# imgag/ngs-bits

Hardware: AMD Instinct MI355X
Metric: Mreads/sec + achieved HBM GB/s, MappingQC 30x WGS BAM at 1/2/4/8 MI355X (higher is better)
Workload: dtype u8/int32/int64

## Files before the change

### ngs-bits_amd/csrc/handle.h

```cpp
#pragma once
#include "common.h"
#include <memory>
#include <condition_variable>
#include <mutex>
#include <algorithm>
#include <cstring>
#include <chrono>
#include <atomic>
#include <functional>
#include <thread>
#include <deque>
#include <fstream>
#include <fcntl.h>
#include <sys/mman.h>
#include <sys/stat.h>
#include <unistd.h>

using namespace ngsqc;

namespace ngsqc { namespace lib {
extern thread_local std::string g_open_error;

struct FormatError : std::runtime_error { using std::runtime_error::runtime_error; };
struct ArgError : std::runtime_error { using std::runtime_error::runtime_error; };
// ... 99 lines not shown

inline uint16_t rd16(const uint8_t* p) { return (uint16_t)(p[0] | (p[1] << 8)); }
inline uint32_t rd32(const uint8_t* p) { return (uint32_t)p[0] | ((uint32_t)p[1] << 8) | ((uint32_t)p[2] << 16) | ((uint32_t)p[3] << 24); }

constexpr int K1_CHUNK_WAVES_PER_CU = 5;
constexpr int P1_WAVES_PER_CU = 10;
constexpr int N_DEPTH_SETS = 2;

struct DepthSet
{
	std::vector<ngsqc_region> regions; std::vector<int64_t> doff; std::vector<int32_t> rlen; int64_t n_slots = 0; int64_t roi_bases = 0;
	DevBuf<int32_t> d_reg_start, d_reg_end, d_reg_len, d_tid_first, d_tid_last; DevBuf<int64_t> d_doff; DevBuf<int32_t> d_depth; DevBuf<uint8_t> d_tmp;
	bool depth_ready = false;
};

struct TileCtx { const uint8_t* infl; int64_t total; const int64_t* recoff; int64_t n_rec; int64_t ord_base; int tile; bool last; };
}}

using namespace ngsqc::lib;

struct ngsqc_handle
{
	const OpenSwitches osw;
	CallSwitches sw;
	std::string err, path;
	bool from_cram = false;
	bool selection = false;
	int device = 0; int n_cu = 256;
	hipStream_t stream = nullptr;
	hipStream_t s_p1[2] = {nullptr, nullptr};
	hipStream_t s_p2 = nullptr;
	hipStream_t s_crc = nullptr;
	size_t csize = 0;
	std::vector<BlockDesc> blocks; int64_t total = 0;
	std::vector<uint32_t> crc;
	std::vector<uint64_t> member_off;
	DevBuf<uint8_t> d_comp;
	std::vector<std::string> ref_names; std::vector<int64_t> ref_lens; int64_t first_rec = 0; std::string header_text;
	bool planned = false;
	int64_t chunk = 0, nch = 0;
	std::vector<std::pair<int64_t, int64_t>> tiles;
	std::vector<int64_t> tile_first_chunk;
	int64_t pfx = 0, max_tile_bytes = 0, slot_pages = 0;
	DevBuf<BlockDesc> d_kdesc;
	DevBuf<uint32_t> d_tok_first, d_tok_cnt, d_order, d_tok, d_crc, d_pool_ctr; DevBuf<unsigned long long> d_work; DevBuf<BlockStatus> d_status;
	int p1_wgs = 0;
	DevBuf<uint32_t> d_sync_pool; DevBuf<BlockDesc> d_sync_desc; DevBuf<uint32_t> d_sync_u32; DevBuf<BlockStatus> d_sync_st; DevBuf<unsigned long long> d_sync_work;
	static constexpr int MAX_TILE_BUFS = 4;
	int k1_slots = osw.token_slots;
	DevBuf<uint8_t> buf[MAX_TILE_BUFS]; int nbuf = 2;
	int64_t max_tile_members = 0;
	std::vector<hipEvent_t> ev_chunk;
	std::vector<hipEvent_t> ev_tile;
	PinBuf<BlockStatus> p_status; PinBuf<int32_t> p_start; PinBuf<int64_t> p_next; PinBuf<unsigned long long> p_small;
	bool decoded = false; int cur_tile = -1;
	int64_t n_rec = 0; DevBuf<int64_t> d_recoff;
	DevBuf<int64_t> d_long;
	int64_t tile_prefix = 0, tile_total = 0, tile_u_lo = 0, tile_ord_base = 0;
	int64_t carry_len = 0, carry_src = 0, next_ord_base = 0, expected_abs = 0;
	int64_t k1_enq = 0;
	DevBuf<int32_t> d_start; DevBuf<uint32_t> d_cnt; DevBuf<int64_t> d_next, d_base; DevBuf<uint32_t> d_bad; DevBuf<uint8_t> d_scan_tmp; DevBuf<uint16_t> d_rel;
	DepthSet ds[N_DEPTH_SETS]; int cur_ds = 0;
	ngsqc_timings tm{};
	int shard = 0, n_shards = 1;
	int64_t shard_own_members = -1;
	int64_t shard_limit = -1;
	int64_t shard_u_base = 0;
	int64_t shard_first_abs = -1, shard_exit_abs = -1; int shard_last_tile = -1;
	bool verify_crc = osw.verify_crc;
	struct Upload
	{
		std::vector<std::thread> th; std::mutex mu; std::condition_variable cv;
		std::vector<hipEvent_t> ev; std::vector<char> recorded; size_t piece = 0, n_pieces = 0, bytes = 0; std::atomic<size_t> next{0}; std::atomic<bool> cancel{false};
		std::string err; void* map = nullptr; size_t map_n = 0; int fd = -1; double t0 = 0, t_done = 0; size_t done = 0;
		size_t waited[4] = {0, 0, 0, 0};
		struct SPiece { size_t src, dst, bytes; int64_t chunk; };
		std::vector<SPiece> sp; std::vector<size_t> chunk_first;
		std::atomic<int64_t> p2_enq{0}; bool pass_running = false, pass_fresh = false; const uint8_t* src_base = nullptr;
	};
	Upload* up = nullptr;
	bool stream_img = false; int comp_slots = 0; size_t comp_slot_bytes = 0;
	std::vector<uint64_t> chunk_lo;
	DevBuf<uint8_t> d_sync_comp;
	std::thread plan_thread; std::string plan_err;
	EvLog ev_store; EvLog* evlog = &ev_store;
	PinBuf<unsigned long long> p_rb; static constexpr int RB_CAND = 64, RB_BQ = 65, RB_TOTAL = 72;
	bool lazy_recoff = false; int recoff_tile = -1;
	struct RecoffArgs { const uint8_t* base = nullptr; int64_t total = 0; const BlockDesc* desc = nullptr; int64_t ne = 0, prefix = 0, n_rec = 0, nm = 0; int ksh = 0; int tile = -1; } rw;
	struct FusedScan
	{
		virtual void fused_launch(ngsqc_handle* h, const uint8_t* infl, int64_t total, int sgn, const BlockDesc* d_desc, int64_t ne, int64_t prefix, int ksh, int64_t nm, int64_t scan_limit) = 0;
		virtual void fused_readback(ngsqc_handle* h) = 0;
		virtual unsigned long long fused_bq_cap() = 0;
		virtual ~FusedScan() = default;
	};
	FusedScan* fuse = nullptr; bool fuse_ok = true; int fused_tile = -1;
	bool long_reads = false;
	int lr_failures = 0;
	bool k2_plain = false;
	std::vector<int64_t> rq_len_hist, rq_cyc;
	struct Partial;
	Partial* partial = nullptr;
};

namespace ngsqc { namespace lib {
inline void dbg_stamp(bool on, const char* what)
{
	static const double t0 = wall_ms();
	if (on) fprintf(stderr, "[ngsqc] t+%.1f ms %s\n", wall_ms() - t0, what);
}

template <typename F> int guarded(ngsqc_handle* h, F f)
{
	if (!h) return NGSQC_E_ARG;
	h->sw = CallSwitches();
	try { HIPCHK(hipSetDevice(h->device)); f(); return NGSQC_OK; }
	catch (FormatError& e) { h->err = e.what(); return NGSQC_E_FORMAT; }
	catch (ArgError& e) { h->err = e.what(); return NGSQC_E_ARG; }
	catch (IoError& e) { h->err = e.what(); return NGSQC_E_IO; }
	catch (std::domain_error& e) { h->err = e.what(); return NGSQC_E_UNSUPPORTED; }
	catch (std::exception& e) { h->err = e.what(); return NGSQC_E_DEVICE; }
}

void walk_bgzf(const uint8_t* file, size_t n, size_t& off, size_t off_end, int64_t max_members, uint64_t& upos, std::vector<BlockDesc>& blocks, std::vector<uint32_t>& crc, std::vector<uint64_t>* file_off = nullptr);
void scan_bgzf(const uint8_t* file, size_t n, std::vector<BlockDesc>& blocks, std::vector<uint32_t>& crc, int64_t& total, std::vector<uint64_t>* file_off, int threads, bool* in_pieces = nullptr);
std::string inflate_error(const ngsqc_handle* h, int64_t member, uint32_t code);
void inflate_sync(ngsqc_handle* h, const std::vector<int64_t>& idx, const std::vector<BlockDesc>& desc, uint8_t* d_out, int level = 0);
void upload_wait(ngsqc_handle* h, size_t end_byte, hipStream_t st, int slot);
void upload_join(ngsqc_handle* h);
void upload_finish(ngsqc_handle* h);
void stream_pass_begin(ngsqc_handle* h);
void stream_pass_end(ngsqc_handle* h);
void stream_wait_chunk(ngsqc_handle* h, int64_t c, hipStream_t st);
void stream_p2_enqueued(ngsqc_handle* h, int64_t c);
void plan_layout(ngsqc_handle* h);
struct RangeRequest { bool by_name = false; uint64_t voff[2] = {0, 0}; const ngsqc_named_region* regions = nullptr; int64_t n_regions = 0; int64_t head_members = 0; };
int open_impl(ngsqc_handle** out, const char* path, const void* bytes, size_t n, int device, int shard = 0, int n_shards = 1, const RangeRequest* range = nullptr);

const int64_t* ensure_recoff(ngsqc_handle* h);
void sync_all(ngsqc_handle* h);
void stream_tiles(ngsqc_handle* h, const std::function<bool(const TileCtx&)>& f);
void for_each_tile(ngsqc_handle* h, const std::function<bool(int)>& f);

constexpr int64_t BGZF_PIECE = 0xff00;
size_t bgzf_max_bytes(int64_t n);
struct BgzfDeflater
{
	DevBuf<uint16_t> prev; DevBuf<uint32_t> tok, sizes; DevBuf<uint64_t> off; DevBuf<uint8_t> slots, scan_tmp;
	int grid = 0; int64_t cap_members = 0;
	void reserve(int64_t max_members, int device);
	size_t run(const uint8_t* d_in, int64_t n, uint8_t* d_out, hipStream_t s, int device, int level = -1);
// ... 5 lines not shown
```

### ngs-bits_amd/csrc/image.hip

```cpp
#include "handle.h"

namespace ngsqc { namespace lib {
void walk_bgzf(const uint8_t* file, size_t n, size_t& off, size_t off_end, int64_t max_members, uint64_t& upos, std::vector<BlockDesc>& blocks, std::vector<uint32_t>& crc, std::vector<uint64_t>* file_off)
{
	int64_t k = 0;
	while (off < n && off < off_end && k < max_members)
	{
		if (off + 18 > n) throw FormatError("truncated BGZF header");
		const uint8_t* p = file + off;
		if (p[0] != 31 || p[1] != 139 || p[2] != 8 || !(p[3] & 4)) throw FormatError("not a BGZF block (gzip member without BC extra field)");
		uint32_t xlen = rd16(p + 10), bsize = 0; bool found = false;
		size_t x = 12, xend = 12 + (size_t)xlen;
		if (off + xend > n) throw FormatError("truncated BGZF extra field");
		while (x + 4 <= xend) { uint16_t slen = rd16(p + x + 2); if (p[x] == 'B' && p[x + 1] == 'C' && slen == 2) { bsize = rd16(p + x + 4) + 1u; found = true; } x += 4 + slen; }
		if (!found || bsize < xend + 8 || off + bsize > n) throw FormatError("invalid BGZF block size");
		uint32_t isize = rd32(p + bsize - 4);
		if (isize > 65536) throw FormatError("BGZF block inflates to more than 64 KiB");
		if (isize) { blocks.push_back(BlockDesc{(uint64_t)(off + xend), upos, (uint32_t)(bsize - xend - 8), isize}); crc.push_back(rd32(p + bsize - 8)); if (file_off) file_off->push_back((uint64_t)off); }
		upos += isize; off += bsize; ++k;
	}
}
uint32_t bgzf_member_at(const uint8_t* file, size_t n, size_t off)
{
	if (off + 18 > n) return 0;
// ... 469 lines not shown
	}
	if (h->nch <= cpt) cpt = h->nch;
	h->tiles.clear(); h->tile_first_chunk.clear();
	for (int64_t c = 0; c < h->nch; c += cpt)
	{
		const int64_t m0 = c * h->chunk, m1 = std::min(nb, (c + cpt) * h->chunk);
		h->tiles.emplace_back(m0, m1 - m0); h->tile_first_chunk.push_back(c);
	}
	h->tile_first_chunk.push_back(h->nch);
	const int nt = (int)h->tiles.size();
	h->pfx = nt > 1 ? ((carry_max + 255) & ~255ll) : 0;
	std::vector<BlockDesc> kd((size_t)nb); h->max_tile_bytes = 0;
	for (int t = 0; t < nt; ++t)
	{
		const int64_t f = h->tiles[(size_t)t].first, m = h->tiles[(size_t)t].second; const uint64_t u_lo = h->blocks[(size_t)f].upos;
		for (int64_t i = f; i < f + m; ++i) { kd[(size_t)i] = h->blocks[(size_t)i]; kd[(size_t)i].upos -= u_lo; }
		h->max_tile_bytes = std::max<int64_t>(h->max_tile_bytes, (int64_t)(h->blocks[(size_t)(f + m - 1)].upos + h->blocks[(size_t)(f + m - 1)].usize - u_lo));
	}
	if (h->stream_img)
	{
		h->comp_slots = (int)std::min<int64_t>(h->osw.comp_slots ? h->osw.comp_slots : 8, h->nch);
		h->chunk_lo.assign((size_t)h->nch, 0); std::vector<uint64_t> chunk_hi((size_t)h->nch, 0); size_t slot = 0;
		for (int64_t c = 0; c < h->nch; ++c)
		{
			const int64_t c0 = c * h->chunk, cn = std::min(h->chunk, nb - c0);
			h->chunk_lo[(size_t)c] = h->blocks[(size_t)c0].cpos & ~15ull;
			chunk_hi[(size_t)c] = std::min<uint64_t>(h->blocks[(size_t)(c0 + cn - 1)].cpos + h->blocks[(size_t)(c0 + cn - 1)].clen + 64, h->up->map_n);
			slot = std::max<size_t>(slot, (size_t)(chunk_hi[(size_t)c] - h->chunk_lo[(size_t)c]));
		}
		h->comp_slot_bytes = (slot + 1024 + 4095) & ~(size_t)4095;
		h->d_comp.alloc((size_t)h->comp_slots * h->comp_slot_bytes + 1024);
		HIPCHK(hipMemsetAsync(h->d_comp.p, 0, (size_t)h->comp_slots * h->comp_slot_bytes + 1024, h->stream));
		const size_t piece = (size_t)h->osw.h2d_piece_mb << 20;
		ngsqc_handle::Upload* u = h->up; u->sp.clear(); u->chunk_first.assign((size_t)h->nch + 1, 0);
		for (int64_t c = 0; c < h->nch; ++c)
		{
			const int64_t c0 = c * h->chunk, cn = std::min(h->chunk, nb - c0);
			const size_t base = (size_t)(c % h->comp_slots) * h->comp_slot_bytes;
			for (int64_t i = c0; i < c0 + cn; ++i) kd[(size_t)i].cpos = base + (h->blocks[(size_t)i].cpos - h->chunk_lo[(size_t)c]);
			u->chunk_first[(size_t)c] = u->sp.size();
			for (uint64_t o = h->chunk_lo[(size_t)c]; o < chunk_hi[(size_t)c]; o += piece)
				u->sp.push_back(ngsqc_handle::Upload::SPiece{(size_t)o, base + (size_t)(o - h->chunk_lo[(size_t)c]), (size_t)std::min<uint64_t>(piece, chunk_hi[(size_t)c] - o), c});
		}
		u->chunk_first[(size_t)h->nch] = u->sp.size();
	}
	h->d_kdesc.upload(kd, h->stream); h->d_order.upload(ord, h->stream); h->d_crc.upload(h->crc, h->stream);
	h->d_tok_cnt.ensure((size_t)nb + 8); h->d_tok_first.ensure((size_t)nb + 8); h->d_status.ensure((size_t)nb); h->d_work.ensure((size_t)h->nch); h->d_pool_ctr.ensure((size_t)h->nch);
	dbg_stamp(h->osw.debug, "layout: member tables on the device");
	h->d_tok.ensure((size_t)(n_slots * h->slot_pages) * K1_PAGE_WORDS + 16);
	dbg_stamp(h->osw.debug, "layout: token pool allocated");
	for (int i = 0; i < std::min(nt, h->nbuf); ++i) h->buf[i].ensure((size_t)(h->pfx + h->max_tile_bytes) + 64);
	dbg_stamp(h->osw.debug, "layout: tile buffers allocated");
	h->max_tile_members = 0; for (auto& tl : h->tiles) h->max_tile_members = std::max(h->max_tile_members, tl.second);
	h->p_status.ensure((size_t)nb);
	while ((int64_t)h->ev_chunk.size() < 4 * h->nch) { hipEvent_t e; HIPCHK(hipEventCreate(&e)); h->ev_chunk.push_back(e); }
	while ((int)h->ev_tile.size() < 2 * nt) { hipEvent_t e; HIPCHK(hipEventCreateWithFlags(&e, hipEventDisableTiming)); h->ev_tile.push_back(e); }
	h->p_small.ensure(64); h->p_rb.ensure((size_t)ngsqc_handle::RB_TOTAL);
	HIPCHK(hipStreamSynchronize(h->stream));
	h->tm.n_tiles = nt;
	if (h->stream_img && early_pass) { stream_pass_begin(h); h->up->pass_fresh = true; }
	if (h->osw.debug) fprintf(stderr, "[ngsqc] layout: %d tiles, %lld chunks, %d image slots, token pool %.1f GB, tile buffers %.1f GB, %.1f ms\n", nt, (long long)h->nch, h->comp_slots, (double)n_slots * (double)h->slot_pages * K1_PAGE_WORDS * 4e-9, (double)std::min(nt, h->nbuf) * (double)(h->pfx + h->max_tile_bytes) * 1e-9, wall_ms() - pl0);
}

void plan_layout(ngsqc_handle* h)
{
	if (h->plan_thread.joinable())
	{
		h->plan_thread.join();
		if (!h->plan_err.empty()) { const std::string e = h->plan_err; h->plan_err.clear(); throw std::runtime_error(e); }
	}
	plan_layout_now(h);
}


void open_range_common(ngsqc_handle* h, const uint8_t* bytes, size_t n, int device, const RangeRequest& rq)
{
	if (n >= 4 && memcmp(bytes, "CRAM", 4) == 0) throw std::domain_error("a CRAM file has no BGZF members: ngsqc_open / ngsqc_open_memory decode it (cram.hip)");
	init_device(h, device);
	Timer t(h->stream); t.start();
	size_t off = 0; uint64_t upos = 0; std::vector<uint64_t> hdr_off;
	for (int64_t k = 8;; k *= 4)
	{
		walk_bgzf(bytes, n, off, n, k - (int64_t)hdr_off.size() > 0 ? k - (int64_t)hdr_off.size() : k, upos, h->blocks, h->crc, &hdr_off);
		const size_t end = h->blocks.empty() ? 0 : (size_t)(h->blocks.back().cpos + h->blocks.back().clen);
		upload_compressed(h, bytes, 0, end);
		h->total = (int64_t)upos;
		if (read_header(h, (int64_t)h->blocks.size())) break;
		if (off >= n) throw FormatError("Could not read header from BAM/CRAM file " + h->path);
	}
	uint64_t beg = rq.voff[0], end = rq.voff[1]; bool found = true;
	uint64_t own_end = 0;
	if (rq.by_name)
	{
		std::vector<ngsqc_region> regs;
		for (int64_t i = 0; i < rq.n_regions; ++i)
		{
			const std::string want = rq.regions[i].chr ? rq.regions[i].chr : "";
			for (size_t r = 0; r < h->ref_names.size(); ++r) if (h->ref_names[r] == want || chr_norm(h->ref_names[r]) == chr_norm(want)) { regs.push_back(ngsqc_region{(int32_t)r, rq.regions[i].start, rq.regions[i].end}); break; }
		}
		if (!bai_range(h->path, regs.data(), (int64_t)regs.size(), (int32_t)h->ref_names.size(), beg, end, found))
			throw IoError("Could not load index of BAM/CRAM file " + h->path);
	}
	if (rq.head_members > 0)
	{
		size_t k = 0; while (k + 1 < h->blocks.size() && (int64_t)(h->blocks[k].upos + h->blocks[k].usize) <= h->first_rec) ++k;
		found = !h->blocks.empty() && h->first_rec < h->total;
		if (!found && off < n) { walk_bgzf(bytes, n, off, n, 1, upos, h->blocks, h->crc, &hdr_off); h->total = (int64_t)upos; k = h->blocks.size() - 1; found = h->first_rec < h->total; }
// ... 127 lines not shown
```

### ngs-bits_amd/csrc/jobs.hip

```cpp
#include "handle.h"

namespace ngsqc { namespace lib {

void setup_regions(ngsqc_handle* h, DepthSet& D, const ngsqc_region* regions, int64_t n, bool with_depth = true)
{
	const int n_ref = (int)h->ref_names.size();
	D.regions.assign(regions, regions + (n > 0 ? n : 0));
	D.doff.assign((size_t)n + 1, 0); D.rlen.assign((size_t)n, 0);
	std::vector<int32_t> rs((size_t)n), re((size_t)n), tf((size_t)std::max(n_ref, 1), 0), tl((size_t)std::max(n_ref, 1), 0);
	std::vector<uint8_t> seen((size_t)std::max(n_ref, 1), 0);
	int64_t slots = 0, bases = 0;
	for (int64_t i = 0; i < n; ++i)
	{
		const ngsqc_region& r = regions[i];
		if (r.tid < 0 || r.tid >= n_ref) throw ArgError("region with invalid reference id");
		if (r.start < 1 || r.end < r.start) throw ArgError("invalid region range");
		if (i > 0 && regions[i - 1].tid == r.tid) { if (regions[i - 1].end >= r.start) throw ArgError("Merged and sorted BED file required for coverage details statistics!"); }
		else { if (seen[r.tid]) throw ArgError("Merged and sorted BED file required for coverage details statistics!"); seen[r.tid] = 1; tf[r.tid] = (int32_t)i; }
		tl[r.tid] = (int32_t)i + 1;
		rs[i] = r.start; re[i] = r.end; D.rlen[i] = r.end - r.start + 1; D.doff[i] = slots;
		slots += (int64_t)D.rlen[i] + 1; bases += D.rlen[i];
	}
	D.doff[n] = slots; D.n_slots = slots; D.roi_bases = bases;
	D.d_reg_start.upload(rs, h->stream); D.d_reg_end.upload(re, h->stream); D.d_reg_len.upload(D.rlen, h->stream);
// ... 627 lines not shown
	{
		map.scan.end(h);
		if (!part)
		{
			Timer fin(h->stream); fin.start();
			finalize_depth(h, h->ds[0]);
			h->tm.finalize_ms = fin.stop();
			mapping_counters(h, map, (int)(map.scan.best_key >> 40), map.scan.first_paired != ~0ull, map.scan.sum_runmax, map.scan.fix_len, r->counters, r->gc_reads);
		}
		else
		{
			const unsigned long long key = map.scan.best_key;
			shard_out->n_records = h->tm.n_records;
			shard_out->first_abs = h->shard_own_members >= 0 ? h->shard_first_abs : (h->tm.n_records ? h->first_rec : -1);
			shard_out->exit_abs = h->shard_own_members >= 0 ? h->shard_exit_abs : (h->tm.n_records ? h->total : -1);
			shard_out->max_len = (int64_t)(key >> 40);
			shard_out->first_max_ord = key ? (int64_t)(0xFFFFFFFFFFull - (key & 0xFFFFFFFFFFull)) : -1;
			shard_out->first_paired_ord = map.scan.first_paired != ~0ull ? (int64_t)map.scan.first_paired : -1;
		}
		h->tm.scan_ms = map.scan.stage_ms; h->tm.scan_kernel_ms = map.scan.kernel_ms; h->tm.scan_launches = map.scan.launches;
	}
	if (do_depth)
	{
		dscan.end(h);
		if (!part) { Timer fin(h->stream); fin.start(); finalize_depth(h, h->ds[1]); h->tm.finalize_ms += fin.stop(); }
		h->tm.depth_scan_ms = dscan.stage_ms;
		if (!do_map) { h->tm.scan_algorithmic_bytes = (int64_t)dscan.dev[A_ALG_BYTES]; h->tm.scan_kernel_ms = dscan.kernel_ms; h->tm.scan_launches = dscan.launches; h->tm.scan_ms = dscan.stage_ms; }
	}
	if (do_sites) { pile.end(h, r->site_counts); h->tm.pileup_ms = pile.stage_ms; }
	if (do_indel) { indel.end(h, ij->counts); h->tm.pileup_ms += indel.stage_ms; }
	if (do_reads) { reads.end(h, r->read_stats); h->tm.reads_ms = reads.stage_ms; }
	h->cur_ds = do_map || !do_depth ? 0 : 1;
	h->tm.total_ms = total.stop();
	h->tm.job_wall_ms = wall_ms() - w0;
	if (h->sw.debug) fprintf(stderr, "[ngsqc] job: setup %.2f ms, tile stream %.2f ms (K1 %.2f), results %.2f ms\n", w1 - w0, w2 - w1, h->tm.inflate_ms, wall_ms() - w2);
}

DepthSet& cur_depth(ngsqc_handle* h) { return h->ds[h->cur_ds]; }

}}

extern "C" {

void ngsqc_close(ngsqc_handle* h)
{
	if (!h) return;
	struct Hold { Hold() { reaper().hold(); } ~Hold() { reaper().unhold(); } } hold_frees;
	if (h->plan_thread.joinable()) h->plan_thread.join();
	if (h->up) { upload_join(h); delete h->up; h->up = nullptr; }
	if (h->stream) { (void)hipSetDevice(h->device); sync_all(h); }
	for (hipStream_t s : {h->stream, h->s_p1[0], h->s_p1[1], h->s_p2, h->s_crc}) if (s) (void)hipStreamDestroy(s);
	for (hipEvent_t e : h->ev_chunk) (void)hipEventDestroy(e);
	for (hipEvent_t e : h->ev_tile) (void)hipEventDestroy(e);
	delete h->partial;
	delete h;
}

int ngsqc_run_job(ngsqc_handle* h, const ngsqc_job_desc* job, ngsqc_job_result* result) { return guarded(h, [&] { run_job(h, job, result); }); }

int ngsqc_depth_select(ngsqc_handle* h, int32_t which)
{
	return guarded(h, [&] { if (which < 0 || which >= N_DEPTH_SETS) throw ArgError("invalid depth set"); h->cur_ds = which; });
}

int ngsqc_scan_mapping(ngsqc_handle* h, const ngsqc_mapping_params* p, int64_t* counters, double* gc_reads)
{
	return guarded(h, [&] {
		if (!p || !counters) throw ArgError("null argument");
		ngsqc_job_desc j{}; j.mapping = p; ngsqc_job_result r{}; r.counters = counters; r.gc_reads = gc_reads;
		run_job(h, &j, &r);
	});
}

int ngsqc_scan_mapping_partial(ngsqc_handle* h, const ngsqc_mapping_params* p, ngsqc_shard_summary* out)
{
	return guarded(h, [&] {
		if (!p || !out) throw ArgError("null argument");
		ngsqc_job_desc j{}; j.mapping = p; ngsqc_job_result r{};
		run_job(h, &j, &r, out);
	});
}
int ngsqc_run_job_partial(ngsqc_handle* h, const ngsqc_job_desc* job, ngsqc_job_result* result, ngsqc_shard_summary* out)
{
	return guarded(h, [&] { if (!out) throw ArgError("null argument"); run_job(h, job, result, out); });
}

int ngsqc_scan_mapping_finish(ngsqc_handle* h, const ngsqc_shard_fix* fix, int64_t* counters, double* gc_reads)
{
	return guarded(h, [&] {
		if (!fix || !counters) throw ArgError("null argument");
		if (!h->partial) throw ArgError("ngsqc_scan_mapping_finish without ngsqc_scan_mapping_partial");
		ngsqc_handle::Partial& st = *h->partial; ScanState& sc = st.scan;
		Timer total(h->stream); total.start();
		const int64_t f = fix->trim_upto, pidx = st.mode != NGSQC_MODE_ROI ? fix->paired_upto : 0;
		unsigned long long fx[4] = {0, 0, (unsigned long long)std::max<int64_t>(fix->floor_max, 0), 0};
		if (f > 0 || pidx > 0)
		{
			HIPCHK(hipMemcpyAsync(sc.d_counters.p + A_FIX_TRIM, fx, sizeof(fx), hipMemcpyHostToDevice, h->stream));
			const int64_t upto = std::max(f, pidx);
			if (upto <= st.head_n)
				launch_prefix_fix(sc.sp, f, pidx, st.d_head.p, h->stream);
			else stream_tiles(h, [&](const TileCtx& c) {
				sc.sp.infl = c.infl; sc.sp.total = c.total; sc.sp.recoff = c.recoff; sc.sp.n_rec = c.n_rec; sc.sp.ord_base = c.ord_base;
				const int64_t lf = std::min<int64_t>(std::max<int64_t>(f - c.ord_base, 0), c.n_rec), lp = std::min<int64_t>(std::max<int64_t>(pidx - c.ord_base, 0), c.n_rec);
				launch_prefix_fix(sc.sp, lf, lp, nullptr, h->stream);
				HIPCHK(hipStreamSynchronize(h->stream));
// ... 324 lines not shown
```

### ngs-bits_amd/csrc/tiles.hip

```cpp
#include "handle.h"

namespace ngsqc { namespace lib {

void enqueue_k1_tile(ngsqc_handle* h, int t)
{
	const int64_t nb = (int64_t)h->blocks.size();
	uint8_t* out_base = h->buf[t % h->nbuf].p + h->pfx;
	const bool k1_serial = h->sw.k1_serial;
	hipStream_t crc_stream = h->s_crc;
	const int64_t cA = h->tile_first_chunk[(size_t)t], cB = h->tile_first_chunk[(size_t)t + 1];
	auto launch_p1 = [&](int64_t c) {
		const int64_t c0 = c * h->chunk, cn = std::min(h->chunk, nb - c0);
		hipEvent_t* e4 = &h->ev_chunk[(size_t)(4 * c)];
		hipStream_t s1 = k1_serial ? h->s_p2 : h->s_p1[c & 1];
		if (c >= h->k1_slots) HIPCHK(hipStreamWaitEvent(s1, h->ev_chunk[(size_t)(4 * (c - h->k1_slots) + 3)], 0));
		if (h->stream_img) stream_wait_chunk(h, c, s1);
		else if (h->up) { const BlockDesc& lb = h->blocks[(size_t)(c0 + cn - 1)]; upload_wait(h, (size_t)(lb.cpos + lb.clen + 64), s1, k1_serial ? 3 : 1 + (int)(c & 1)); }
		HIPCHK(hipEventRecord(e4[0], s1));
		uint32_t* const pool = h->d_tok.p + (size_t)(c % h->k1_slots) * (size_t)h->slot_pages * K1_PAGE_WORDS;
		launch_huff_tokens(h->d_comp.p, h->d_kdesc.p + c0, cn, h->d_status.p + c0, pool, (uint32_t)h->slot_pages, h->d_pool_ctr.p + c, h->d_tok_first.p + c0, h->d_tok_cnt.p + c0, h->d_work.p + c,
		                   h->d_order.p + c0, h->p1_wgs, h->osw.p1_park, s1);
		HIPCHK(hipEventRecord(e4[1], s1));
	};
	auto launch_p2 = [&](int64_t c) {
		const int64_t c0 = c * h->chunk, cn = std::min(h->chunk, nb - c0);
		hipEvent_t* e4 = &h->ev_chunk[(size_t)(4 * c)];
		uint32_t* const pool = h->d_tok.p + (size_t)(c % h->k1_slots) * (size_t)h->slot_pages * K1_PAGE_WORDS;
		HIPCHK(hipStreamWaitEvent(h->s_p2, e4[1], 0));
		if (c == cA && t >= h->nbuf) HIPCHK(hipStreamWaitEvent(h->s_p2, h->ev_tile[(size_t)(2 * (t - h->nbuf) + 1)], 0));
		HIPCHK(hipEventRecord(e4[2], h->s_p2));
		launch_lz77_resolve(h->d_kdesc.p + c0, cn, out_base, h->d_status.p + c0, pool, h->d_tok_first.p + c0, h->d_tok_cnt.p + c0, h->d_comp.p, h->s_p2);
		HIPCHK(hipEventRecord(e4[3], h->s_p2));
		if (h->stream_img) stream_p2_enqueued(h, c);
		if (h->verify_crc)
		{
			if (crc_stream != h->s_p2) HIPCHK(hipStreamWaitEvent(crc_stream, e4[3], 0));
			launch_crc32(h->d_kdesc.p + c0, cn, out_base, h->d_crc.p + c0, h->d_status.p + c0, h->sw.crc_chains, crc_stream);
		}
	};
	for (int64_t c = cA; c < cB; ++c) { launch_p1(c); launch_p2(c); }
	const int64_t f = h->tiles[(size_t)t].first, m = h->tiles[(size_t)t].second;
	hipStream_t s_last = h->verify_crc ? crc_stream : h->s_p2;
	HIPCHK(hipMemcpyAsync(h->p_status.p + f, h->d_status.p + f, (size_t)m * sizeof(BlockStatus), hipMemcpyDeviceToHost, s_last));
	HIPCHK(hipEventRecord(h->ev_tile[(size_t)(2 * t)], s_last));
	h->tm.inflate_launches++;
	h->k1_enq = h->tile_first_chunk[(size_t)t + 1];
}

void finish_k1_tile(ngsqc_handle* h, int t)
{
	HIPCHK(hipEventSynchronize(h->ev_tile[(size_t)(2 * t)]));
	const int64_t f = h->tiles[(size_t)t].first, m = h->tiles[(size_t)t].second;
	std::vector<int64_t> redo;
	for (int64_t i = f; i < f + m; ++i)
	{
		const uint32_t e = h->p_status.p[i].error;
		if (e == K1_ERR_TOKEN_OVERFLOW) redo.push_back(i);
		else if (e) throw FormatError(inflate_error(h, i, e));
	}
	h->tm.members_inflated += m;
	if (redo.empty()) return;
	std::vector<BlockDesc> desc; const uint64_t u_lo = h->blocks[(size_t)f].upos;
	for (int64_t i : redo) { BlockDesc d = h->blocks[(size_t)i]; d.upos -= u_lo; desc.push_back(d); }
	inflate_sync(h, redo, desc, h->buf[t % h->nbuf].p + h->pfx);
}

const int64_t* ensure_recoff(ngsqc_handle* h)
{
	const ngsqc_handle::RecoffArgs& a = h->rw;
	if (h->recoff_tile != a.tile || a.tile < 0)
	{
		h->d_recoff.ensure_slack((size_t)std::max<int64_t>(a.n_rec, 1));
		size_t iv = h->evlog->begin(h->stream, &h->tm.index_ms);
		launch_index_write(a.base, a.total, a.desc, a.ne, a.prefix, a.ksh, a.nm, h->d_start.p, h->d_cnt.p, h->d_base.p, h->d_rel.p, h->d_recoff.p, h->stream);
		h->evlog->end(iv, h->stream);
		h->recoff_tile = a.tile;
	}
	return h->d_recoff.p;
}

void index_tile(ngsqc_handle* h, int t)
{
	const bool dbg = h->sw.debug;
	const int nt = (int)h->tiles.size();
	const bool last = t == nt - 1;
	const int64_t first = h->tiles[(size_t)t].first, nm = h->tiles[(size_t)t].second;
	if (t == 0) { h->carry_len = 0; h->next_ord_base = 0; h->expected_abs = h->first_rec; }
	const int64_t u_lo = (int64_t)h->blocks[(size_t)first].upos;
	const int64_t u_hi = (int64_t)h->blocks[(size_t)(first + nm - 1)].upos + h->blocks[(size_t)(first + nm - 1)].usize;
	const int64_t prefix = h->carry_len;
	const int64_t total = prefix + (u_hi - u_lo);
	const uint8_t* base = h->buf[t % h->nbuf].p + h->pfx - prefix;
	const BlockDesc* d_desc = h->d_kdesc.p + first;
	const bool anchor_by_guess = t == 0 && h->first_rec < 0;
	int64_t exp0 = prefix ? 0 : (h->expected_abs - u_lo);
	if (t == 0)
	{
		h->long_reads = false;
		const int elr = h->sw.long_read_mode;
		if (elr != SW_UNSET) h->long_reads = elr != 0 && !anchor_by_guess;
		else if (!anchor_by_guess && exp0 >= 0 && exp0 + 4 <= total)
		{
			int64_t off = exp0, sum = 0; int n = 0;
			for (; n < 8 && off + 4 <= total; ++n)
			{
				uint32_t bs = 0;
				HIPCHK(hipMemcpyAsync(&bs, base + off, 4, hipMemcpyDeviceToHost, h->stream)); HIPCHK(hipStreamSynchronize(h->stream));
				if (bs < 32 || bs > (1u << 30)) break;
				sum += bs; off += 4 + (int64_t)bs;
			}
			h->long_reads = n > 0 && sum / n > 8192;
		}
		h->lr_failures = 0;
	}
	int ksh = h->sw.walker_shift;
	if (h->long_reads) ksh = h->sw.group_shift == SW_UNSET ? K2_MIN_KSH : -h->sw.group_shift;
	if (anchor_by_guess || (h->k2_plain && !h->long_reads)) ksh = 0;
	const int64_t ne0 = nm + 1;
	int64_t ne = ksh >= 0 ? (nm << ksh) + 1 : ((nm + (1ll << -ksh) - 1) >> -ksh) + 1;
	auto e_lo = [&](int64_t e) -> int64_t { return e == 0 ? 0 : prefix + ((int64_t)h->blocks[(size_t)(first + e - 1)].upos - u_lo); };
	auto e_sz = [&](int64_t e) -> int64_t { return e == 0 ? prefix : (int64_t)h->blocks[(size_t)(first + e - 1)].usize; };
	EvLog& ev = *h->evlog; size_t iv = ev.begin(h->stream, &h->tm.index_ms);
	const size_t ne_max = (size_t)std::max(ne, ne0);
	h->d_start.ensure_slack(ne_max); h->d_cnt.ensure_slack(ne_max + 1); h->d_next.ensure_slack(ne_max + 1); h->d_base.ensure_slack(ne_max + 1); h->d_bad.ensure(4);
	h->d_scan_tmp.ensure_slack(scan_tmp_bytes((int64_t)ne_max) + 64); h->d_rel.ensure_slack((size_t)(ne0 + 1) * K2_REL_STRIDE + 64);
	int64_t from = 0; int rounds = 0; int64_t straddle = -1; bool found_start = !anchor_by_guess; int64_t chain_exit = total;
	const bool tail_may_cut_a_record = h->shard_own_members >= 0 && h->shard + 1 < h->n_shards;
	const bool assume0 = !anchor_by_guess && !h->k2_plain && !h->long_reads;
	launch_index_init(d_desc, ne, prefix, ksh, nm, exp0, anchor_by_guess, assume0, h->d_start.p, h->stream);
	HIPCHK(hipMemsetAsync(h->d_bad.p, 0, 2 * sizeof(uint32_t), h->stream)); HIPCHK(hipMemsetAsync(h->d_bad.p + 2, 0xff, sizeof(long long), h->stream));
	h->fused_tile = -1;
	const bool try_fuse = h->fuse && (h->fuse_ok || h->long_reads) && !anchor_by_guess && (prefix == 0 || h->long_reads) && !h->sw.no_fused_scan;
	const int64_t fuse_limit = h->shard_own_members >= 0 ? prefix + (h->shard_limit - u_lo) : INT64_MAX;
	if (try_fuse)
	{
		h->d_long.ensure_slack((size_t)std::max<int64_t>(total / 160, 1024));
		if (!assume0 || ksh > 0) launch_index_guess(base, total, d_desc, ne, prefix, ksh, nm, 0, h->d_start.p, (int32_t)h->ref_names.size(), h->stream);
		ev.end(iv, h->stream);
		h->fuse->fused_launch(h, base, total, +1, d_desc, ne, prefix, ksh, nm, fuse_limit);
		iv = ev.begin(h->stream, &h->tm.index_ms);
	}
	else launch_index_count(base, total, d_desc, ne, prefix, ksh, nm, 0, h->d_start.p, h->d_cnt.p, h->d_next.p, h->d_bad.p, (int32_t)h->ref_names.size(), h->d_rel.p, h->stream, !assume0 || ksh > 0);
	launch_index_chain(d_desc, ne, prefix, ksh, nm, exp0, total, h->d_start.p, h->d_next.p, h->d_bad.p + 1, (long long*)(h->d_bad.p + 2), h->stream);
	launch_scan_counts(h->d_cnt.p, ne, h->d_base.p, h->d_scan_tmp.p, h->stream);
	unsigned long long* sm = h->p_small.p + 32;
	HIPCHK(hipMemcpyAsync(sm, h->d_bad.p, 4 * sizeof(uint32_t), hipMemcpyDeviceToHost, h->stream));
	HIPCHK(hipMemcpyAsync(sm + 3, h->d_base.p + ne, sizeof(int64_t), hipMemcpyDeviceToHost, h->stream));
	sm[2] = 0; if (try_fuse) h->fuse->fused_readback(h);
	HIPCHK(hipStreamSynchronize(h->stream));
	if (try_fuse) sm[2] = h->p_rb.p[A_LONG_COUNT];
	const uint32_t n_corrupt = ((const uint32_t*)sm)[0], n_viol = ((const uint32_t*)sm)[1];
	const bool aligned = !anchor_by_guess && n_viol == 0 && !h->sw.k2_general;
	if (try_fuse)
	{
		const bool lists_fit = sm[2] <= (unsigned long long)h->d_long.n && h->p_rb.p[ngsqc_handle::RB_BQ] <= h->fuse->fused_bq_cap();
		if (aligned && n_corrupt == 0 && lists_fit) h->fused_tile = t;
		else if (!aligned || n_corrupt == 0)
		{
			ev.end(iv, h->stream);
			h->fuse->fused_launch(h, base, total, -1, d_desc, ne, prefix, ksh, nm, fuse_limit);
			iv = ev.begin(h->stream, &h->tm.index_ms);
			if (!aligned) h->fuse_ok = false; else h->d_long.ensure_slack((size_t)sm[2]);
		}
	}
	if (aligned)
	{
		if (n_corrupt) throw FormatError("Could not read next alignment in BAM/CRAM file " + h->path + " (corrupt record chain)");
		h->lr_failures = 0;
		straddle = (int64_t)sm[1]; h->tm.tiles_chain_on_device++; if (h->fused_tile == t) h->tm.tiles_scan_fused++;
		h->tm.walkers_per_member = ksh >= 0 ? 1ll << ksh : -(1ll << -ksh);
		if (straddle >= 0 && last && !tail_may_cut_a_record) throw FormatError("Could not read next alignment in BAM/CRAM file " + h->path + " (truncated record)");
		chain_exit = std::max(total, exp0);
	}
	else
	{
	if (!anchor_by_guess) h->k2_plain = true;
	if (h->long_reads && ++h->lr_failures >= 3) h->long_reads = false;
	if (ksh != 0 || assume0)
	{
		ksh = 0; ne = ne0;
		launch_index_init(d_desc, ne, prefix, ksh, nm, exp0, anchor_by_guess, false, h->d_start.p, h->stream);
		HIPCHK(hipMemsetAsync(h->d_bad.p, 0, 2 * sizeof(uint32_t), h->stream));
		launch_index_count(base, total, d_desc, ne, prefix, ksh, nm, 0, h->d_start.p, h->d_cnt.p, h->d_next.p, h->d_bad.p, (int32_t)h->ref_names.size(), h->d_rel.p, h->stream);
	}
	h->p_start.ensure((size_t)ne + 64); h->p_next.ensure((size_t)ne + 64);
	int32_t* start = h->p_start.p; int64_t* next = h->p_next.p;
	bool first_round = true;
	while (true)
	{
		if (!first_round)
		{
			HIPCHK(hipMemsetAsync(h->d_bad.p, 0, sizeof(uint32_t), h->stream));
			launch_index_count(base, total, d_desc, ne, prefix, 0, nm, from, h->d_start.p, h->d_cnt.p, h->d_next.p, h->d_bad.p, (int32_t)h->ref_names.size(), h->d_rel.p, h->stream);
		}
		first_round = false;
		HIPCHK(hipMemcpyAsync(start + from, h->d_start.p + from, (size_t)(ne - from) * sizeof(int32_t), hipMemcpyDeviceToHost, h->stream));
		HIPCHK(hipMemcpyAsync(next + from, h->d_next.p + from, (size_t)(ne - from) * sizeof(int64_t), hipMemcpyDeviceToHost, h->stream));
		HIPCHK(hipStreamSynchronize(h->stream));
		int64_t expected = exp0; int64_t mismatch = -1; straddle = -1; bool anchored = !anchor_by_guess;
		for (int64_t b = 0; b < ne; ++b)
		{
			const int64_t lo = e_lo(b), hi = lo + e_sz(b);
			if (!anchored)
			{
				if (start[b] < 0) continue;
				anchored = true; expected = lo + start[b]; exp0 = expected;
			}
			const int32_t want = expected >= hi ? -1 : (int32_t)(expected - lo);
			if (start[b] != want) { mismatch = b; start[b] = want; break; }
			if (want >= 0)
			{
				const int64_t nx = next[b];
				if (nx == -2) throw FormatError("Could not read next alignment in BAM/CRAM file " + h->path + " (corrupt record chain)");
// ... 43 lines not shown
			else if (straddle < 0 && last) exit_local = total;
			if (!found_start && last) { h->shard_exit_abs = -1; h->shard_last_tile = t; n_rec = 0; straddle = -1; }
			else if (exit_local >= 0 || last)
			{
				if (exit_local < 0) throw FormatError("a record at the end of shard " + std::to_string(h->shard) + " is longer than the members read behind the shard (raise NGSQC_SHARD_TAIL_MEMBERS)");
				h->shard_exit_abs = h->shard_u_base + u_lo + (exit_local - prefix); h->shard_last_tile = t;
				if (lo < n_rec || (straddle >= 0 && straddle >= lim)) straddle = -1;
				n_rec = lo;
			}
		}
	}
	ev.end(iv, h->stream);
	h->cur_tile = t; h->tile_prefix = prefix; h->tile_total = total; h->tile_u_lo = u_lo; h->tile_ord_base = h->next_ord_base;
	h->n_rec = n_rec; h->tm.n_records += n_rec;
	h->carry_src = straddle; h->carry_len = straddle >= 0 ? total - straddle : 0;
	if (h->carry_len > h->pfx && !last) throw FormatError("a record that straddles two tiles is larger than the carry area (" + std::to_string(h->carry_len) + " > " + std::to_string(h->pfx) + " bytes; raise NGSQC_CARRY_MAX)");
	h->expected_abs = u_lo + (chain_exit - prefix);
	h->next_ord_base = h->tile_ord_base + n_rec;
	h->decoded = true;
}

TileCtx resident_ctx(ngsqc_handle* h)
{
	const int nt = (int)h->tiles.size(); const int t = h->cur_tile;
	return TileCtx{h->buf[t % h->nbuf].p + h->pfx - h->tile_prefix, h->tile_total, h->recoff_tile == t ? h->d_recoff.p : nullptr , h->n_rec, h->tile_ord_base, t, t == nt - 1};
}

void reset_decode_timings(ngsqc_handle* h)
{
	h->tm.inflate_ms = 0; h->tm.index_ms = 0; h->tm.inflate_launches = 0; h->tm.n_records = 0; h->tm.inflate_huff_ms = 0; h->tm.inflate_lz77_ms = 0;
	h->tm.inflate_huff_launches = 0; h->tm.members_inflated = 0; h->tm.tiles_chain_on_device = 0; h->tm.tiles_scan_fused = 0;
}

void sync_all(ngsqc_handle* h)
{
	(void)hipStreamSynchronize(h->s_p1[0]); (void)hipStreamSynchronize(h->s_p1[1]); (void)hipStreamSynchronize(h->s_p2); (void)hipStreamSynchronize(h->s_crc); (void)hipStreamSynchronize(h->stream);
}

void stream_tiles(ngsqc_handle* h, const std::function<bool(const TileCtx&)>& f)
{
	plan_layout(h);
	dbg_stamp(h->sw.debug, "tile stream: layout ready");
	const int nt = (int)h->tiles.size();
	if (nt == 0) { h->decoded = true; h->n_rec = 0; return; }
	if (nt == 1 && h->decoded && h->cur_tile == 0)
	{
		try { if (!h->lazy_recoff) ensure_recoff(h); f(resident_ctx(h)); } catch (...) { h->evlog->discard(); throw; }
		h->evlog->resolve(); return;
	}
	reset_decode_timings(h);
	h->decoded = false; h->cur_tile = -1; h->k1_enq = 0; h->k2_plain = false;
	const bool dbg = h->sw.debug;
	const bool pipelined = h->sw.pipeline;
	HIPCHK(hipMemsetAsync(h->d_work.p, 0, (size_t)h->nch * sizeof(unsigned long long), h->stream));
	HIPCHK(hipMemsetAsync(h->d_pool_ctr.p, 0, (size_t)h->nch * sizeof(uint32_t), h->stream));
	HIPCHK(hipStreamSynchronize(h->stream));
	if (h->stream_img)
	{
		if (!(h->up->pass_running && h->up->pass_fresh)) stream_pass_begin(h);
		h->up->pass_fresh = false;
	}
	try
	{
		const int ahead = pipelined ? h->nbuf - 1 : 0;
		for (int u = 0; u < std::min(nt, std::max(1, ahead)); ++u) enqueue_k1_tile(h, u);
		for (int t = 0; t < nt; ++t)
		{
			const double d0 = wall_ms();
			if (pipelined && t + ahead < nt) enqueue_k1_tile(h, t + ahead);
			const double d1 = wall_ms();
			finish_k1_tile(h, t);
			const double d2 = wall_ms();
			index_tile(h, t);
			const double d3 = wall_ms();
			const bool go_on = f(resident_ctx(h));
			if (dbg) fprintf(stderr, "[ngsqc] tile %d/%d: enqueue next K1 %.2f ms, wait K1 %.2f ms, K2 %.2f ms, consumers %.2f ms (%lld records)\n", t, nt, d1 - d0, d2 - d1, d3 - d2, wall_ms() - d3, (long long)h->n_rec);
			const bool stop = !go_on || t == h->shard_last_tile;
			if (!stop && t + 1 < nt && h->carry_len > 0)
				HIPCHK(hipMemcpyAsync(h->buf[(t + 1) % h->nbuf].p + h->pfx - h->carry_len, h->buf[t % h->nbuf].p + h->pfx - h->tile_prefix + h->carry_src, (size_t)h->carry_len, hipMemcpyDeviceToDevice, h->stream));
			HIPCHK(hipEventRecord(h->ev_tile[(size_t)(2 * t + 1)], h->stream));
			if (stop) { if (t + 1 < nt) { sync_all(h); h->decoded = nt == 1; } break; }
			if (!pipelined && t + 1 < nt) { HIPCHK(hipStreamSynchronize(h->stream)); enqueue_k1_tile(h, t + 1); }
		}
	}
	catch (...) { if (h->stream_img) stream_pass_end(h); sync_all(h); h->evlog->discard(); h->decoded = false; h->cur_tile = -1; throw; }
	h->evlog->resolve();
	if (h->stream_img)
	{
		if (h->k1_enq < h->nch) stream_pass_end(h);
		else { upload_finish(h); stream_pass_end(h); }
	}
	if (h->k1_enq > 0)
	{
		const int64_t c_end = h->k1_enq;
		HIPCHK(hipEventSynchronize(h->ev_chunk[(size_t)(4 * (c_end - 1) + 3)]));
		float ms = 0;
		HIPCHK(hipEventElapsedTime(&ms, h->ev_chunk[0], h->ev_chunk[(size_t)(4 * (c_end - 1) + 3)])); h->tm.inflate_ms = ms;
		for (int64_t c = 0; c < c_end; ++c)
		{
			hipEvent_t* e4 = &h->ev_chunk[(size_t)(4 * c)];
			HIPCHK(hipEventElapsedTime(&ms, e4[0], e4[1])); h->tm.inflate_huff_ms += ms;
			HIPCHK(hipEventElapsedTime(&ms, e4[2], e4[3])); h->tm.inflate_lz77_ms += ms;
		}
		h->tm.inflate_huff_launches = c_end;
	}
	if (nt > 1) { h->decoded = false; }
}

void for_each_tile(ngsqc_handle* h, const std::function<bool(int)>& f) { stream_tiles(h, [&](const TileCtx&) { return f(h->cur_tile); }); }
}}
```

Measured before the change: 1168.

## Defer CRC verification off critical path and launch fused walk before host K1 check

When CRC checking is on and tiles are pipelined, the inflate status readback for a tile now waits only on the inflate stream, and CRC results are copied separately and checked after the tile's consumers run. The fused record-chain walk can also be queued on the device as soon as the tile's last chunk event fires, before the host inspects inflate status. If members need redoing, the walk is undone and run again. The aim is to take host synchronisation and CRC latency out of the per-tile critical path, at the cost of more complex error ordering and possible repeated walks.

```diff
diff --git a/ngs-bits_amd/csrc/handle.h b/ngs-bits_amd/csrc/handle.h
--- a/ngs-bits_amd/csrc/handle.h
+++ b/ngs-bits_amd/csrc/handle.h
@@ -175,7 +175,9 @@
 	int64_t max_tile_members = 0;
 	std::vector<hipEvent_t> ev_chunk;
 	std::vector<hipEvent_t> ev_tile;
+	std::vector<hipEvent_t> ev_crc;
 	PinBuf<BlockStatus> p_status; PinBuf<int32_t> p_start; PinBuf<int64_t> p_next; PinBuf<unsigned long long> p_small;
+	PinBuf<BlockStatus> p_crc_status; bool crc_late = false; int crc_confirmed = -1;
 	bool decoded = false; int cur_tile = -1;
 	int64_t n_rec = 0; DevBuf<int64_t> d_recoff;
 	DevBuf<int64_t> d_long;
@@ -220,6 +222,7 @@
 	FusedScan* fuse = nullptr; bool fuse_ok = true; int fused_tile = -1;
 	bool long_reads = false;
 	int lr_failures = 0;
+	bool walk_early = false;
 	bool k2_plain = false;
 	std::vector<int64_t> rq_len_hist, rq_cyc;
 	struct Partial;
diff --git a/ngs-bits_amd/csrc/image.hip b/ngs-bits_amd/csrc/image.hip
--- a/ngs-bits_amd/csrc/image.hip
+++ b/ngs-bits_amd/csrc/image.hip
@@ -545,7 +545,8 @@
 	for (int i = 0; i < std::min(nt, h->nbuf); ++i) h->buf[i].ensure((size_t)(h->pfx + h->max_tile_bytes) + 64);
 	dbg_stamp(h->osw.debug, "layout: tile buffers allocated");
 	h->max_tile_members = 0; for (auto& tl : h->tiles) h->max_tile_members = std::max(h->max_tile_members, tl.second);
-	h->p_status.ensure((size_t)nb);
+	h->p_status.ensure((size_t)nb); if (h->verify_crc) h->p_crc_status.ensure((size_t)nb);
+	while ((int)h->ev_crc.size() < nt) { hipEvent_t e; HIPCHK(hipEventCreateWithFlags(&e, hipEventDisableTiming)); h->ev_crc.push_back(e); }
 	while ((int64_t)h->ev_chunk.size() < 4 * h->nch) { hipEvent_t e; HIPCHK(hipEventCreate(&e)); h->ev_chunk.push_back(e); }
 	while ((int)h->ev_tile.size() < 2 * nt) { hipEvent_t e; HIPCHK(hipEventCreateWithFlags(&e, hipEventDisableTiming)); h->ev_tile.push_back(e); }
 	h->p_small.ensure(64); h->p_rb.ensure((size_t)ngsqc_handle::RB_TOTAL);
diff --git a/ngs-bits_amd/csrc/jobs.hip b/ngs-bits_amd/csrc/jobs.hip
--- a/ngs-bits_amd/csrc/jobs.hip
+++ b/ngs-bits_amd/csrc/jobs.hip
@@ -703,6 +703,7 @@
 	for (hipStream_t s : {h->stream, h->s_p1[0], h->s_p1[1], h->s_p2, h->s_crc}) if (s) (void)hipStreamDestroy(s);
 	for (hipEvent_t e : h->ev_chunk) (void)hipEventDestroy(e);
 	for (hipEvent_t e : h->ev_tile) (void)hipEventDestroy(e);
+	for (hipEvent_t e : h->ev_crc) (void)hipEventDestroy(e);
 	delete h->partial;
 	delete h;
 }
diff --git a/ngs-bits_amd/csrc/tiles.hip b/ngs-bits_amd/csrc/tiles.hip
--- a/ngs-bits_amd/csrc/tiles.hip
+++ b/ngs-bits_amd/csrc/tiles.hip
@@ -40,14 +40,34 @@
 	};
 	for (int64_t c = cA; c < cB; ++c) { launch_p1(c); launch_p2(c); }
 	const int64_t f = h->tiles[(size_t)t].first, m = h->tiles[(size_t)t].second;
-	hipStream_t s_last = h->verify_crc ? crc_stream : h->s_p2;
-	HIPCHK(hipMemcpyAsync(h->p_status.p + f, h->d_status.p + f, (size_t)m * sizeof(BlockStatus), hipMemcpyDeviceToHost, s_last));
-	HIPCHK(hipEventRecord(h->ev_tile[(size_t)(2 * t)], s_last));
+	if (h->crc_late)
+	{
+		HIPCHK(hipMemcpyAsync(h->p_status.p + f, h->d_status.p + f, (size_t)m * sizeof(BlockStatus), hipMemcpyDeviceToHost, h->s_p2));
+		HIPCHK(hipEventRecord(h->ev_tile[(size_t)(2 * t)], h->s_p2));
+		HIPCHK(hipMemcpyAsync(h->p_crc_status.p + f, h->d_status.p + f, (size_t)m * sizeof(BlockStatus), hipMemcpyDeviceToHost, crc_stream));
+		HIPCHK(hipEventRecord(h->ev_crc[(size_t)t], crc_stream));
+	}
+	else
+	{
+		hipStream_t s_last = h->verify_crc ? crc_stream : h->s_p2;
+		HIPCHK(hipMemcpyAsync(h->p_status.p + f, h->d_status.p + f, (size_t)m * sizeof(BlockStatus), hipMemcpyDeviceToHost, s_last));
+		HIPCHK(hipEventRecord(h->ev_tile[(size_t)(2 * t)], s_last));
+	}
 	h->tm.inflate_launches++;
 	h->k1_enq = h->tile_first_chunk[(size_t)t + 1];
 }
 
-void finish_k1_tile(ngsqc_handle* h, int t)
+void confirm_k1_tile(ngsqc_handle* h, int t, int64_t upto = -1)
+{
+	if (!h->crc_late || h->crc_confirmed >= t) return;
+	HIPCHK(hipEventSynchronize(h->ev_crc[(size_t)t]));
+	const int64_t f = h->tiles[(size_t)t].first, end = upto >= 0 ? upto : f + h->tiles[(size_t)t].second;
+	const BlockStatus* st = h->p_crc_status.p;
+	for (int64_t i = f; i < end; ++i) if (st[i].error == K1_ERR_CRC) throw FormatError(inflate_error(h, i, K1_ERR_CRC));
+	if (upto < 0) h->crc_confirmed = t;
+}
+
+std::vector<int64_t> check_k1_tile(ngsqc_handle* h, int t)
 {
 	HIPCHK(hipEventSynchronize(h->ev_tile[(size_t)(2 * t)]));
 	const int64_t f = h->tiles[(size_t)t].first, m = h->tiles[(size_t)t].second;
@@ -56,11 +76,21 @@
 	{
 		const uint32_t e = h->p_status.p[i].error;
 		if (e == K1_ERR_TOKEN_OVERFLOW) redo.push_back(i);
-		else if (e) throw FormatError(inflate_error(h, i, e));
+		else if (e == K1_ERR_CRC && h->crc_late) continue;
+		else if (e)
+		{
+			confirm_k1_tile(h, t, i); h->crc_confirmed = t;
+			throw FormatError(inflate_error(h, i, e));
+		}
 	}
 	h->tm.members_inflated += m;
+	if (!redo.empty()) confirm_k1_tile(h, t);
+	return redo;
+}
+void redo_k1_members(ngsqc_handle* h, int t, const std::vector<int64_t>& redo)
+{
 	if (redo.empty()) return;
-	std::vector<BlockDesc> desc; const uint64_t u_lo = h->blocks[(size_t)f].upos;
+	std::vector<BlockDesc> desc; const uint64_t u_lo = h->blocks[(size_t)h->tiles[(size_t)t].first].upos;
 	for (int64_t i : redo) { BlockDesc d = h->blocks[(size_t)i]; d.upos -= u_lo; desc.push_back(d); }
 	inflate_sync(h, redo, desc, h->buf[t % h->nbuf].p + h->pfx);
 }
@@ -82,6 +112,12 @@
 void index_tile(ngsqc_handle* h, int t)
 {
 	const bool dbg = h->sw.debug;
+	bool k1_waited = false;
+	auto finish_k1 = [&]() { if (!k1_waited) { k1_waited = true; redo_k1_members(h, t, check_k1_tile(h, t)); } };
+	bool early = h->walk_early && h->fuse && h->fuse_ok && !h->k2_plain && !h->sw.no_fused_scan && !h->sw.k2_general && h->sw.walker_shift == 0 && h->shard_own_members < 0
+	                && (t == 0 || h->carry_len == 0) && !(t == 0 && h->first_rec < 0) && (t == 0 ? h->sw.long_read_mode != 1 : !h->long_reads);
+	if (!early) finish_k1();
+	const int64_t cA = h->tile_first_chunk[(size_t)t], cB = h->tile_first_chunk[(size_t)t + 1];
 	const int nt = (int)h->tiles.size();
 	const bool last = t == nt - 1;
 	const int64_t first = h->tiles[(size_t)t].first, nm = h->tiles[(size_t)t].second;
@@ -101,13 +137,25 @@
 		if (elr != SW_UNSET) h->long_reads = elr != 0 && !anchor_by_guess;
 		else if (!anchor_by_guess && exp0 >= 0 && exp0 + 4 <= total)
 		{
-			int64_t off = exp0, sum = 0; int n = 0;
-			for (; n < 8 && off + 4 <= total; ++n)
-			{
-				uint32_t bs = 0;
-				HIPCHK(hipMemcpyAsync(&bs, base + off, 4, hipMemcpyDeviceToHost, h->stream)); HIPCHK(hipStreamSynchronize(h->stream));
-				if (bs < 32 || bs > (1u << 30)) break;
-				sum += bs; off += 4 + (int64_t)bs;
+			int64_t off = 0, sum = 0; int n = 0;
+			auto sample = [&](int64_t lim) {
+				off = exp0; sum = 0; n = 0;
+				for (; n < 8 && off + 4 <= lim; ++n)
+				{
+					uint32_t bs = 0;
+					HIPCHK(hipMemcpyAsync(&bs, base + off, 4, hipMemcpyDeviceToHost, h->stream)); HIPCHK(hipStreamSynchronize(h->stream));
+					if (bs < 32 || bs > (1u << 30)) break;
+					sum += bs; off += 4 + (int64_t)bs;
+				}
+			};
+			if (k1_waited) sample(total);
+			else
+			{
+				const BlockDesc& lb = h->blocks[(size_t)(std::min(first + nm, (cA + 1) * h->chunk) - 1)];
+				const int64_t lim0 = (int64_t)(lb.upos + lb.usize) - u_lo;
+				HIPCHK(hipStreamWaitEvent(h->stream, h->ev_chunk[(size_t)(4 * cA + 3)], 0));
+				sample(lim0);
+				if (n < 8 && off + 4 > lim0 && lim0 < total) { early = false; finish_k1(); sample(total); }
 			}
 			h->long_reads = n > 0 && sum / n > 8192;
 		}
@@ -132,12 +180,29 @@
 	h->fused_tile = -1;
 	const bool try_fuse = h->fuse && (h->fuse_ok || h->long_reads) && !anchor_by_guess && (prefix == 0 || h->long_reads) && !h->sw.no_fused_scan;
 	const int64_t fuse_limit = h->shard_own_members >= 0 ? prefix + (h->shard_limit - u_lo) : INT64_MAX;
+	early = early && try_fuse && assume0 && ksh == 0 && prefix == 0;
+	if (!early) finish_k1();
+	auto walk_tile = [&](int sgn) { h->fuse->fused_launch(h, base, total, sgn, d_desc, ne, prefix, ksh, nm, fuse_limit); };
 	if (try_fuse)
 	{
 		h->d_long.ensure_slack((size_t)std::max<int64_t>(total / 160, 1024));
 		if (!assume0 || ksh > 0) launch_index_guess(base, total, d_desc, ne, prefix, ksh, nm, 0, h->d_start.p, (int32_t)h->ref_names.size(), h->stream);
 		ev.end(iv, h->stream);
-		h->fuse->fused_launch(h, base, total, +1, d_desc, ne, prefix, ksh, nm, fuse_limit);
+		if (early)
+		{
+			HIPCHK(hipStreamWaitEvent(h->stream, h->ev_chunk[(size_t)(4 * (cB - 1) + 3)], 0));
+			walk_tile(+1);
+			k1_waited = true;
+			const std::vector<int64_t> redo = check_k1_tile(h, t);
+			if (!redo.empty())
+			{
+				walk_tile(-1);
+				redo_k1_members(h, t, redo);
+				HIPCHK(hipMemsetAsync(h->d_bad.p, 0, 2 * sizeof(uint32_t), h->stream));
+				walk_tile(+1);
+			}
+		}
+		else walk_tile(+1);
 		iv = ev.begin(h->stream, &h->tm.index_ms);
 	}
 	else launch_index_count(base, total, d_desc, ne, prefix, ksh, nm, 0, h->d_start.p, h->d_cnt.p, h->d_next.p, h->d_bad.p, (int32_t)h->ref_names.size(), h->d_rel.p, h->stream, !assume0 || ksh > 0);
@@ -158,7 +223,7 @@
 		else if (!aligned || n_corrupt == 0)
 		{
 			ev.end(iv, h->stream);
-			h->fuse->fused_launch(h, base, total, -1, d_desc, ne, prefix, ksh, nm, fuse_limit);
+			walk_tile(-1);
 			iv = ev.begin(h->stream, &h->tm.index_ms);
 			if (!aligned) h->fuse_ok = false; else h->d_long.ensure_slack((size_t)sm[2]);
 		}
@@ -308,6 +373,9 @@
 	h->decoded = false; h->cur_tile = -1; h->k1_enq = 0; h->k2_plain = false;
 	const bool dbg = h->sw.debug;
 	const bool pipelined = h->sw.pipeline;
+	h->crc_late = h->verify_crc && pipelined && !h->sw.k1_serial && h->fuse != nullptr; h->crc_confirmed = -1;
+	if (h->crc_late) h->p_crc_status.ensure(h->blocks.size());
+	h->walk_early = pipelined && !h->sw.k1_serial;
 	HIPCHK(hipMemsetAsync(h->d_work.p, 0, (size_t)h->nch * sizeof(unsigned long long), h->stream));
 	HIPCHK(hipMemsetAsync(h->d_pool_ctr.p, 0, (size_t)h->nch * sizeof(uint32_t), h->stream));
 	HIPCHK(hipStreamSynchronize(h->stream));
@@ -325,12 +393,11 @@
 			const double d0 = wall_ms();
 			if (pipelined && t + ahead < nt) enqueue_k1_tile(h, t + ahead);
 			const double d1 = wall_ms();
-			finish_k1_tile(h, t);
-			const double d2 = wall_ms();
-			index_tile(h, t);
-			const double d3 = wall_ms();
-			const bool go_on = f(resident_ctx(h));
-			if (dbg) fprintf(stderr, "[ngsqc] tile %d/%d: enqueue next K1 %.2f ms, wait K1 %.2f ms, K2 %.2f ms, consumers %.2f ms (%lld records)\n", t, nt, d1 - d0, d2 - d1, d3 - d2, wall_ms() - d3, (long long)h->n_rec);
+			bool go_on = true; double d3 = d1;
+			try { index_tile(h, t); d3 = wall_ms(); go_on = f(resident_ctx(h)); }
+			catch (...) { confirm_k1_tile(h, t); throw; }
+			confirm_k1_tile(h, t);
+			if (dbg) fprintf(stderr, "[ngsqc] tile %d/%d: enqueue next K1 %.2f ms, wait K1 + K2 %.2f ms, consumers %.2f ms (%lld records)\n", t, nt, d1 - d0, d3 - d1, wall_ms() - d3, (long long)h->n_rec);
 			const bool stop = !go_on || t == h->shard_last_tile;
 			if (!stop && t + 1 < nt && h->carry_len > 0)
 				HIPCHK(hipMemcpyAsync(h->buf[(t + 1) % h->nbuf].p + h->pfx - h->carry_len, h->buf[t % h->nbuf].p + h->pfx - h->tile_prefix + h->carry_src, (size_t)h->carry_len, hipMemcpyDeviceToDevice, h->stream));
```

New measurement: 1186, median of 6. +1.5%, better.
